# scenarios/VAE-2

Hardware: AMD Instinct MI355X
Metric: training frames/sec on 128x256 8-frame Cityscapes clips, 1/2/4/8 MI355X (higher is better)
Workload: dtype fp32; 1 GPU; VAE2 ELBO step (encz + encoder + 2 decoders fwd/bwd + Adam), HRNet-W18-small-v2, 128x256, 8 clips/GPU x 9 frames (CLIP_LENGTH=3); yaml=vae-2_amd/experiments/vae2_w18_small_v2_128x256.yaml, global_batch=8, frames_per_clip=9, parallelism=dp1, sync_bn=False, launch=hip_graph, mfma_operands=fp32

## Files before the change

### vae-2_amd/csrc/build.py

```python
import concurrent.futures as cf
import os
import shutil
import subprocess
import sys

HERE = os.path.dirname(os.path.abspath(__file__))
PKG = os.path.join(os.path.dirname(HERE), "vae2")
TAG = os.environ.get("VAE2_BUILD_TAG", "")
DEFS = os.environ.get("VAE2_DEFS", "").split()
OUT = os.path.join(PKG, f"libvae2_hip_{TAG}.so" if TAG else "libvae2_hip.so")
BUILD = os.path.join(HERE, f"build_{TAG}" if TAG else "build")
SOURCES = ["conv.hip", "bn.hip", "resample.hip", "elbo.hip", "heads.hip", "clips.hip",
           "metrics.hip", "wgrad_narrow.hip", "syncbn.hip", "dconv_stream.hip"]
HEADERS = ["common.h", os.path.join("..", "..", "include", "vae2_hip.h")]
ARCH = os.environ.get("VAE2_OFFLOAD_ARCH", "gfx950")
FLAGS = ["-O3", "-std=c++17", "-fPIC", f"--offload-arch={ARCH}", "-Wall",
         "-Wno-unused-function", "-munsafe-fp-atomics"]
EXTRA = {"conv.hip": ["-fno-slp-vectorize"], "dconv_stream.hip": ["-fno-slp-vectorize"]}
PARTS = {"conv.hip": 4}


def _units():
    out = []
    for src in SOURCES:
        n = PARTS.get(src, 0)
        base = os.path.splitext(src)[0]
        if n:
            out += [(src, f"{base}_p{i}.o", [f"-DVAE2_CONV_PART={i}"]) for i in range(n)]
        else:
            out.append((src, base + ".o", []))
    return out


def hipcc():
    for cand in (os.environ.get("HIPCC"), "/opt/rocm/bin/hipcc", shutil.which("hipcc")):
        if cand and os.path.exists(cand):
            return cand
    raise RuntimeError("hipcc not found (set HIPCC)")


def _newer(target, deps):
    if not os.path.exists(target):
        return True
    t = os.path.getmtime(target)
    return any(os.path.getmtime(d) > t for d in deps)


def _compile(unit):
    src, oname, defs = unit
    obj = os.path.join(BUILD, oname)
    deps = [os.path.join(HERE, src)] + [os.path.join(HERE, h) for h in HEADERS]
    if not _newer(obj, deps):
        return obj, None
    cmd = [hipcc()] + FLAGS + EXTRA.get(src, []) + defs + DEFS + ["-c", os.path.join(HERE, src), "-o", obj]
    r = subprocess.run(cmd, capture_output=True, text=True)
    if r.returncode != 0:
        return obj, f"$ {' '.join(cmd)}\n{r.stdout}\n{r.stderr}"
    return obj, None


def build(verbose=True, force=False):
    os.makedirs(BUILD, exist_ok=True)
    if force:
        for f in os.listdir(BUILD):
            os.remove(os.path.join(BUILD, f))
    units = _units()
    with cf.ThreadPoolExecutor(max_workers=min(8, len(units))) as ex:
        results = list(ex.map(_compile, units))
    errors = [e for _, e in results if e]
    if errors:
        raise RuntimeError("HIP compile failed:\n" + "\n".join(errors))
    objs = [o for o, _ in results]
    if force or _newer(OUT, objs):
        cmd = [hipcc(), "-shared", "-fPIC", f"--offload-arch={ARCH}", "-o", OUT] + objs
        r = subprocess.run(cmd, capture_output=True, text=True)
        if r.returncode != 0:
            raise RuntimeError(f"link failed:\n$ {' '.join(cmd)}\n{r.stdout}\n{r.stderr}")
    if verbose:
        print(f"built {OUT}")
    return OUT


if __name__ == "__main__":
    build(force="--force" in sys.argv)
```

### vae-2_amd/csrc/common.h

```cpp
#pragma once

#include <hip/hip_runtime.h>
#include <stdint.h>
#include <string>
#include <stdio.h>

#include "../../include/vae2_hip.h"

namespace vae2 {

constexpr int kSyncMaxRanks = 8;

void set_error(const std::string& msg);
int fail(const char* fn, const std::string& msg);
int check_launch(const char* fn);

void note_kernel(const void* host_fn);
#define VAE2_LAUNCH(K, ...)                                         \
  do {                                                              \
    ::vae2::note_kernel(reinterpret_cast<const void*>(K));          \
    hipLaunchKernelGGL(K, __VA_ARGS__);                             \
  } while (0)

#define VAE2_REQUIRE(cond, fn, msg)          \
// ... 95 lines not shown
inline int64_t act_pixels(const vae2_act* d) { return d->n * d->h * d->w; }
inline int64_t act_elems(const vae2_act* d) { return d->n * d->h * d->w * d->c; }

constexpr int kWave = 64;

__device__ __forceinline__ float wave_sum(float v) {
#pragma unroll
  for (int o = 32; o > 0; o >>= 1) v += __shfl_xor(v, o, 64);
  return v;
}

__device__ __forceinline__ double wave_sum_d(double v) {
#pragma unroll
  for (int o = 32; o > 0; o >>= 1) v += __shfl_xor(v, o, 64);
  return v;
}

inline int64_t ceil_div(int64_t a, int64_t b) { return (a + b - 1) / b; }

struct FastDiv {
  uint32_t d, m, s;
  FastDiv() : d(1), m(0), s(0) {}
  explicit FastDiv(uint32_t div) : d(div) {
    for (s = 0; s < 32; ++s)
      if ((1u << s) >= d) break;
    uint64_t one = 1;
    m = (uint32_t)(((one << 32) * ((one << s) - d)) / d + 1);
  }
  __device__ __forceinline__ uint32_t div(uint32_t n) const {
    return (__umulhi(n, m) + n) >> s;
  }
};

struct Lerp {
  int i0, i1;
  float l0, l1;
};

__device__ __forceinline__ Lerp lerp_index(int dst, int in_size, float scale) {
  float src = scale * ((float)dst + 0.5f) - 0.5f;
  if (src < 0.f) src = 0.f;
  int i0 = (int)src;
  if (i0 > in_size - 1) i0 = in_size - 1;
  int ip = (i0 < in_size - 1) ? 1 : 0;
  Lerp l;
  l.i0 = i0;
  l.i1 = i0 + ip;
  l.l1 = src - (float)i0;
  l.l0 = 1.f - l.l1;
  return l;
}

__device__ __forceinline__ float lerp_weight(int o, int in_size, float scale, int i) {
  Lerp l = lerp_index(o, in_size, scale);
  float w = 0.f;
  if (l.i0 == i) w += l.l0;
  if (l.i1 == i) w += l.l1;
  return w;
}

__device__ constexpr float hat_w(int d, int f) {
  return 1.f - (float)(2 * d + 1 - f < 0 ? f - 1 - 2 * d : 2 * d + 1 - f) / (float)(2 * f);
}

int adj3_fuse_launch(const float* dy, const vae2_act* dyd, int n, float* const* dxs,
                     const vae2_act* dxds, const float* betas, hipStream_t st);
extern int g_relu_dual_q;

int64_t wgrad3n_splits(const vae2_act* xd, const vae2_act* dyd);
int wgrad3n_launch(const float* x, const vae2_act* xd, const float* dy, const vae2_act* dyd,
                   float* part, const float* isave, int irelu, uint32_t x_bytes,
                   uint32_t dy_bytes, hipStream_t s);

extern int g_dconv_stream, g_dconv_stream_wpc, g_dconv_stream_bl, g_dconv_stream_spb,
    g_wgrad_narrow_tps, g_bn_blocks, g_bn_apply_res, g_fuse_quad;
bool dconv3s_shape(const vae2_act* ad, const vae2_act* yd);
int64_t dconv3s_rows(const vae2_act* ad, const vae2_act* yd);
int dconv3s_launch(const float* a, const vae2_act* ad, const float* wp, uint32_t w_bytes,
                   const float* bias, float* y, const vae2_act* yd, float beta, float* stats,
                   bool flip, const float* isave, int irelu, const float* bx, int bx_ps,
                   int brelu, const float* bsave, uint32_t bx_bytes, uint32_t a_bytes,
                   hipStream_t s);

int bias_grad_from_partials(const float* partials, int64_t rows, int64_t c,
                            float* dbias, int accumulate, void* stream);

inline unsigned ew_blocks(int64_t n, int threads = 256, int64_t cap = 65536) {
  int64_t b = ceil_div(n, threads);
  if (b > cap) b = cap;
  if (b < 1) b = 1;
  return (unsigned)b;
}

}
```

### vae-2_amd/csrc/conv.hip

```cpp
#include <mutex>
#include <vector>

#include "common.h"

#ifndef VAE2_ABLATE
#define VAE2_ABLATE 0
#endif

#ifndef VAE2_CONV_PART
#define VAE2_CONV_PART -1
#endif
#define VAE2_PART(n) (VAE2_CONV_PART < 0 || VAE2_CONV_PART == (n))

namespace vae2 {


static inline int round_up(int a, int b) { return (a + b - 1) / b * b; }

#if VAE2_PART(0)
__global__ void pack_weight_kernel(const float* __restrict__ w, int cout, int cin, int kk,
                                   int mode, int ld, float* __restrict__ out) {
  const int rows = mode == 0 ? (cout + 63) / 64 * 64 : (cin + 63) / 64 * 64;
  const int cols4 = mode == 0 ? (cin + 3) / 4 * 4 : (cout + 3) / 4 * 4;
  const int total = rows * kk * cols4;
// ... 2633 lines not shown
  const char* fn = "vae2_conv2d_pack_weight";
  VAE2_REQUIRE(w && out && cout > 0 && cin > 0 && k > 0 && (mode == 0 || mode == 1), fn,
               "bad arguments");
  VAE2_REQUIRE(ld >= cin * k * k && ld < (int64_t(1) << 31), fn, "bad row stride");
  int64_t total = vae2_conv2d_packed_size(cout, cin, k, mode);
  VAE2_LAUNCH(pack_weight_kernel, dim3(ew_blocks(total, 256, 2048)), dim3(256), 0,
                     as_stream(stream), w, (int)cout, (int)cin, k * k, mode, (int)ld, out);
  return check_launch(fn);
}

int vae2_conv2d_pack_weight(const float* w, int64_t cout, int64_t cin, int k, int mode,
                            float* out, void* stream) {
  return vae2_conv2d_pack_weight_ld(w, cout, cin, k, mode, cin * k * k, out, stream);
}

int vae2_conv2d_pack_weights(const vae2_pack_job* jobs, int64_t njobs, void* stream) {
  const char* fn = "vae2_conv2d_pack_weights";
  VAE2_REQUIRE(jobs && njobs > 0 && njobs <= 65535, fn, "bad job table");
  VAE2_LAUNCH(pack_weights_batched_kernel, dim3(32, (unsigned)njobs), dim3(256), 0,
                     as_stream(stream), jobs);
  return check_launch(fn);
}

int vae2_conv2d_set_tune(int key, int value) {
  if (key == 0) {
    const int prev = g_igemm_minblk;
    g_igemm_minblk = value < 0 ? 0 : value;
    return prev;
  }
  if (key == 1) {
    const int prev = g_wgrad_cols;
    g_wgrad_cols = value ? 1 : 0;
    return prev;
  }
  if (key == 2) {
    const int prev = g_dconv_nw8;
    g_dconv_nw8 = value ? 1 : 0;
    return prev;
  }
  if (key == 3) {
    const int prev = g_wgrad_nw8;
    g_wgrad_nw8 = value ? 1 : 0;
    return prev;
  }
  if (key == 4) {
    if (value < 3 || value > 8) return -1;
    const int prev = g_gemm1_tn;
    g_gemm1_tn = value;
    return prev;
  }
  if (key == 5) {
    const int prev = g_gemm1_tm;
    g_gemm1_tm = value == 1 ? 1 : 2;
    return prev;
  }
  if (key == 6) {
    if (value < 0 || value > 2) return -1;
    const int prev = g_igemm_nr;
    g_igemm_nr = value;
    return prev;
  }
  if (key == 8) {
    const int prev = g_bn_v2;
    g_bn_v2 = value ? 1 : 0;
    return prev;
  }
  if (key == 7) {
    if (value < 0 || value > 3) return -1;
    const int prev = g_wgrad_narrow;
    g_wgrad_narrow = value;
    return prev;
  }
  if (key == 9) {
    const int prev = g_dconv_stream;
    g_dconv_stream = value >= 0 && value <= 3 ? value : 3;
    return prev;
  }
  if (key == 18) {
    if (value < 256 || value > 8192) return -1;
    const int prev = g_wgrad_wgs;
    g_wgrad_wgs = value;
    return prev;
  }
  if (key == 21) {
    const int prev = g_fuse_quad;
    g_fuse_quad = value ? 1 : 0;
    return prev;
  }
  if (key == 20) {
    if (value < 0 || value > 65536) return -1;
    const int prev = g_bn_apply_res;
    g_bn_apply_res = value;
    return prev;
  }
  if (key == 19) {
    if (value < 256 || value > 8192) return -1;
    const int prev = g_bn_blocks;
    g_bn_blocks = value;
    return prev;
  }
  if (key == 16) {
    if (value < 1 || value > 2) return -1;
    const int prev = g_wgrad_narrow_tps;
    g_wgrad_narrow_tps = value;
    return prev;
  }
  if (key == 17) {
    if (value < 1 || value > 2) return -1;
    const int prev = g_dconv_stream_spb;
    g_dconv_stream_spb = value;
    return prev;
  }
  if (key == 15) {
    if (value < 0 || value > 2) return -1;
    const int prev = g_dconv_ksp;
    g_dconv_ksp = value;
    return prev;
  }
  if (key == 14) {
    const int prev = g_dconv_split72;
    g_dconv_split72 = value ? 1 : 0;
    return prev;
  }
  if (key == 13) {
    const int prev = g_dconv_n16;
    g_dconv_n16 = value ? 1 : 0;
    return prev;
  }
  if (key == 12) {
    const int prev = g_igemm_tab;
    g_igemm_tab = value ? 1 : 0;
    return prev;
  }
  if (key == 11) {
    const int prev = g_dconv_stream_bl;
    g_dconv_stream_bl = value ? 1 : 0;
    return prev;
  }
  if (key == 10) {
    const int prev = g_dconv_stream_wpc;
    g_dconv_stream_wpc = value >= 0 && value <= 8 ? value : 0;
    return prev;
  }
  return -1;
}

int vae2_conv2d_set_mfma_bf16(int on) {
  const int prev = g_bf16;
  g_bf16 = on ? 1 : 0;
  return prev;
}

#endif

#if VAE2_PART(3)
int vae2_wgrad_defer(int on) {
  const int prev = g_wr_defer ? 1 : 0;
  g_wr_defer = on != 0;
  return prev;
}

static int wgrad_flush_impl(void* stream, bool own_only) {
  const char* fn = "vae2_wgrad_flush";
  hipStream_t want = as_stream(stream);
  std::vector<WRQueued> q;
  {
    std::lock_guard<std::mutex> lk(g_wr_mu);
    if (own_only) {
      std::vector<WRQueued> keep;
      for (const WRQueued& j : g_wr_queue) (j.stream == want ? q : keep).push_back(j);
      g_wr_queue.swap(keep);
    } else {
      q.swap(g_wr_queue);
    }
  }
  size_t i = 0;
  while (i < q.size()) {
    WRMulti m{};
    hipStream_t st = want;
    int blocks = 0;
    while (i < q.size() && m.n < kWrMaxJobs) {
      WRJob j = q[i].job;
      const float* lo = j.dw;
      const float* hi = j.dw + (int64_t)(j.cout - 1) * j.ld + (int64_t)j.cin * j.k * j.k;
      bool clash = false;
      for (int u = 0; u < m.n; ++u) {
        const float* lo2 = m.j[u].dw;
        const float* hi2 = m.j[u].dw + (int64_t)(m.j[u].cout - 1) * m.j[u].ld +
                           (int64_t)m.j[u].cin * m.j[u].k * m.j[u].k;
        if (lo < hi2 && lo2 < hi) clash = true;
      }
      if (clash) break;
      j.blk0 = blocks;
      blocks += (int)ceil_div((int64_t)j.cout * j.k * j.k * j.cin4, 32);
      m.j[m.n++] = j;
      ++i;
    }
    VAE2_LAUNCH(wgrad_reduce_multi_kernel, dim3((unsigned)blocks), dim3(256), 0, st, m);
    const int rc = check_launch(fn);
    if (rc) return rc;
  }
  return 0;
}

int vae2_wgrad_flush(void* stream) { return wgrad_flush_impl(stream, false); }

int vae2_wgrad_flush_stream(void* stream) { return wgrad_flush_impl(stream, true); }



#endif

#if VAE2_PART(0)
int vae2_conv2d_set_algo(int algo) {
  const int prev = g_conv_algo + (g_wide_tiles ? 0 : 4) + (g_ksplit ? 0 : 8) +
                   (g_dconv_nr ? 0 : 16) + (g_gemm1 ? 0 : 32) + (g_vec_out ? 0 : 64) +
                   (g_dconv_nr_wide ? 0 : 128);
  const int a = algo & 7;
  if (algo >= 0 && algo <= 255 && a <= 6 && a != 3) {
    g_dconv_nr_wide = (algo & 128) ? 0 : 1;
    g_conv_algo = a & 3;
    g_wide_tiles = a < 4;
    g_ksplit = !(algo & 8);
    g_dconv_nr = !(algo & 16);
    g_gemm1 = !(algo & 32);
    g_vec_out = !(algo & 64);
  }
  return prev;
}

int64_t vae2_conv2d_fwd_stats_rows(const float* x, const vae2_act* xd, const vae2_act* yd,
                                   int k, int stride, int pad) {
  if (!act_ok(xd) || !act_ok(yd)) return 0;
  if (dconv_use(xd, yd, k, stride, pad, x)) return dconv_rows(xd, yd);
  G1Tile g1;
  if (gemm1_pick(xd, yd, k, stride, pad, x, &g1)) return g1.grid_x;
  return igemm_rows(act_pixels(yd), (int)yd->c, k * k, round_up((int)xd->c, 4));
}

int vae2_conv2d_fwd_kernel_name(const vae2_act* xd, const vae2_act* yd, int k, int stride,
                                int pad, char* buf, int64_t len) {
  if (!xd || !yd || !buf || len <= 0) return -22;
  if (dconv_use(xd, yd, k, stride, pad, (const float*)16)) {
    if (stream_use(xd, yd)) {
      const int q = (int)((xd->c + 3) / 4);
      snprintf(buf, (size_t)len, "dconv3s_kernel<%d, %d, %d, false", q == 5 ? 1 : 2,
               q == 5 ? 2 : 4, q);
      return 0;
    }
    DTile d = pick_dtile(xd, yd);
    if (d.nr)
      snprintf(buf, (size_t)len, "dconv3_kernel<%d, %d, false, false, %d>", d.tm, d.tn, d.nr);
    else
      snprintf(buf, (size_t)len, "dconv3_kernel<%d, %d, false>", d.tm, d.tn);
    return 0;
  }
  G1Tile g1;
  if (gemm1_pick(xd, yd, k, stride, pad, (const float*)16, &g1)) {
    snprintf(buf, (size_t)len, "gemm1x1_kernel<%d, %d>", g1.tm, g1.tn);
    return 0;
  }
  Tile t = pick_igemm_tile(act_pixels(yd), (int)yd->c, k * k, round_up((int)xd->c, 4), 1);
  if (t.ks > 1)
    snprintf(buf, (size_t)len, "igemm_kernel<%d, %d, true, 0, %d>", t.tm, t.tn, t.ks);
  else
    snprintf(buf, (size_t)len, "igemm_kernel<%d, %d, true, 0>", t.tm, t.tn);
  return 0;
}

int vae2_conv2d_fwd(const float* x, const vae2_act* xd, const float* wp,
                    const float* bias, float* y, const vae2_act* yd, int k,
                    int stride, int pad, float beta, float* stats,
                    void* stream) {
  const char* fn = "vae2_conv2d_fwd";
  VAE2_REQUIRE(x && wp && y, fn, "null pointer");
  VAE2_REQUIRE(conv_shapes_ok(xd, yd, k, stride, pad), fn, "inconsistent conv shapes");
  VAE2_REQUIRE(fits32(xd) && fits32(yd), fn, "tensor too large for 32-bit indexing");
  if (dconv_use(xd, yd, k, stride, pad, x)) {
    return launch_dconv(x, xd, wp, (uint32_t)(vae2_conv2d_packed_size(yd->c, xd->c, k, 0) * 4),
                        bias, y, yd, beta, stats, false, as_stream(stream), fn);
  }
  G1Tile g1;
  if (gemm1_pick(xd, yd, k, stride, pad, x, &g1)) {
    const int rc = launch_gemm1(x, xd, wp,
                                (uint32_t)(vae2_conv2d_packed_size(yd->c, xd->c, k, 0) * 4),
                                bias, y, yd, beta, stats, g1, as_stream(stream), fn);
    if (rc != -1) return rc;
    VAE2_REQUIRE(stats == nullptr, fn, "BN statistics need a 16-byte aligned output here");
  }
  IGemm p{};
  p.a = x; p.a_ps = (int)xd->ps; p.a_c = (int)xd->c; p.a_c4 = round_up((int)xd->c, 4);
  p.a_h = (int)xd->h; p.a_w = (int)xd->w;
  p.g_n = (int)yd->n; p.g_h = (int)yd->h; p.g_w = (int)yd->w;
  p.a_step = stride;
  p.nth = k; p.ntw = k;
  p.dh0 = -pad; p.dhs = 1; p.dw0 = -pad; p.dws = 1;
  p.kh0 = 0; p.khs = 1; p.kw0 = 0; p.kws = 1; p.ksz = k;
  p.w = wp; p.n = (int)yd->c;
  p.a_bytes = act_bytes(xd);
  p.w_bytes = (uint32_t)(vae2_conv2d_packed_size(yd->c, xd->c, k, 0) * 4);
  p.bias = bias;
  p.y = y; p.y_ps = (int)yd->ps; p.y_h = (int)yd->h; p.y_w = (int)yd->w;
  p.y_step = 1; p.y_offh = 0; p.y_offw = 0;
  p.beta = beta;
  p.stats = stats;
  return launch_igemm(p, 0, as_stream(stream), fn);
}

int vae2_conv2d_bnin_ok(const float* x, const vae2_act* xd, const vae2_act* yd, int k,
                        int stride, int pad) {
  if (!x || !conv_shapes_ok(xd, yd, k, stride, pad) || !fits32(xd) || !fits32(yd)) return 0;
  return !g_bf16 && dconv_use(xd, yd, k, stride, pad, x) && g_conv_algo != 1 &&
         wgrad3_shape_ok(xd, yd, k, stride, pad) && vec_ok(x, (int)xd->ps);
}

int vae2_conv2d_fwd_bnin(const float* x, const vae2_act* xd, const float* bn_save, int relu,
                         const float* wp, const float* bias, float* y, const vae2_act* yd,
                         int k, int stride, int pad, float beta, float* stats, void* stream) {
  const char* fn = "vae2_conv2d_fwd_bnin";
  VAE2_REQUIRE(x && wp && y && bn_save, fn, "null pointer");
  VAE2_REQUIRE(conv_shapes_ok(xd, yd, k, stride, pad), fn, "inconsistent conv shapes");
  VAE2_REQUIRE(vae2_conv2d_bnin_ok(x, xd, yd, k, stride, pad), fn,
               "input BatchNorm needs the direct 3x3 kernels (vae2_conv2d_bnin_ok)");
  BnSide bn;
  bn.isave = bn_save;
  bn.irelu = relu ? 1 : 0;
  return launch_dconv(x, xd, wp, (uint32_t)(vae2_conv2d_packed_size(yd->c, xd->c, k, 0) * 4),
                      bias, y, yd, beta, stats, false, as_stream(stream), fn, bn);
}

static int igemm_dgrad_setup(IGemm& p, const float* dy, const vae2_act* dyd, const float* wp,
                             float* dx, const vae2_act* dxd, int k, int stride, int pad,
                             float beta);
static int64_t igemm_dgrad_rows(const float* dy, const vae2_act* dyd, const vae2_act* dxd,
                                int k, int stride, int pad);

int64_t vae2_conv2d_bwd_data_bnpart_rows(const float* dy, const vae2_act* dyd,
                                         const vae2_act* dxd, int k, int stride, int pad) {
  if (!dy || !conv_shapes_ok(dxd, dyd, k, stride, pad) || !fits32(dxd) || !fits32(dyd))
    return 0;
  if (g_bf16) return 0;
  if (dconv_use(dyd, dxd, k, stride, pad, dy)) return dconv_rows(dyd, dxd);
  G1Tile g1;
  if (gemm1_pick(dyd, dxd, k, stride, pad, dy, &g1)) return g1.grid_x;
  return igemm_dgrad_rows(dy, dyd, dxd, k, stride, pad);
}

int vae2_conv2d_bwd_data_bnpart(const float* dy, const vae2_act* dyd, const float* wp,
                                float* dx, const vae2_act* dxd, int k, int stride, int pad,
                                const float* bn_x, const vae2_act* bn_xd, const float* bn_save,
                                int relu, float* partials, void* stream) {
  const char* fn = "vae2_conv2d_bwd_data_bnpart";
  VAE2_REQUIRE(dy && wp && dx && bn_x && bn_xd && bn_save && partials, fn, "null pointer");
  VAE2_REQUIRE(conv_shapes_ok(dxd, dyd, k, stride, pad), fn, "inconsistent conv shapes");
  VAE2_REQUIRE(bn_xd->n == dxd->n && bn_xd->h == dxd->h && bn_xd->w == dxd->w &&
               bn_xd->c == dxd->c && bn_xd->ps >= bn_xd->c && fits32(bn_xd), fn,
               "BatchNorm input shape must match dx");
  VAE2_REQUIRE(vae2_conv2d_bwd_data_bnpart_rows(dy, dyd, dxd, k, stride, pad) > 0, fn,
               "BatchNorm partials are not available for this geometry "
               "(vae2_conv2d_bwd_data_bnpart_rows)");
  const uint32_t wbytes = (uint32_t)(vae2_conv2d_packed_size(dyd->c, dxd->c, k, 1) * 4);
  if (dconv_use(dyd, dxd, k, stride, pad, dy)) {
    BnSide bn;
    bn.bx = bn_x;
    bn.bx_ps = (int)bn_xd->ps;
    bn.bx_bytes = act_bytes(bn_xd);
    bn.bsave = bn_save;
    bn.brelu = relu ? 1 : 0;
    return launch_dconv(dy, dyd, wp, wbytes, nullptr, dx, dxd, 0.f, partials, true,
                        as_stream(stream), fn, bn);
  }
  G1Tile g1;
  if (gemm1_pick(dyd, dxd, k, stride, pad, dy, &g1)) {
    const int rc = launch_gemm1(dy, dyd, wp, wbytes, nullptr, dx, dxd, 0.f, partials, g1,
                                as_stream(stream), fn, bn_x, (int)bn_xd->ps, relu ? 1 : 0,
                                bn_save, act_bytes(bn_xd));
    VAE2_REQUIRE(rc != -1, fn, "1x1 GEMM refused the partials form");
    return rc;
  }
  IGemm p{};
  const int ncls = igemm_dgrad_setup(p, dy, dyd, wp, dx, dxd, k, stride, pad, 0.f);
  VAE2_REQUIRE(ncls > 0, fn, "stride > 2 is not supported");
  p.stats = partials;
  p.bx = bn_x;
  p.bx_ps = (int)bn_xd->ps;
  p.bx_bytes = act_bytes(bn_xd);
  p.bsave = bn_save;
  p.brelu = relu ? 1 : 0;
  return launch_igemm(p, 1, as_stream(stream), fn, ncls);
}

int vae2_conv2d_bwd_data(const float* dy, const vae2_act* dyd, const float* wp,
                         float* dx, const vae2_act* dxd, int k, int stride,
                         int pad, float beta, void* stream) {
  const char* fn = "vae2_conv2d_bwd_data";
  VAE2_REQUIRE(dy && wp && dx, fn, "null pointer");
  VAE2_REQUIRE(conv_shapes_ok(dxd, dyd, k, stride, pad), fn, "inconsistent conv shapes");
  VAE2_REQUIRE(fits32(dxd) && fits32(dyd), fn, "tensor too large for 32-bit indexing");
  if (dconv_use(dyd, dxd, k, stride, pad, dy))
    return launch_dconv(dy, dyd, wp, (uint32_t)(vae2_conv2d_packed_size(dyd->c, dxd->c, k, 1) * 4),
                        nullptr, dx, dxd, beta, nullptr, true, as_stream(stream), fn);
  G1Tile g1;
  if (gemm1_pick(dyd, dxd, k, stride, pad, dy, &g1)) {
    const int rc = launch_gemm1(dy, dyd, wp,
                                (uint32_t)(vae2_conv2d_packed_size(dyd->c, dxd->c, k, 1) * 4),
                                nullptr, dx, dxd, beta, nullptr, g1, as_stream(stream), fn);
    if (rc != -1) return rc;
  }
  IGemm p{};
  const int ncls = igemm_dgrad_setup(p, dy, dyd, wp, dx, dxd, k, stride, pad, beta);
  VAE2_REQUIRE(ncls >= 0, fn, "stride > 2 is not supported");
  if (ncls == 0) return 0;
  return launch_igemm(p, 1, as_stream(stream), fn, ncls);
}

static int igemm_dgrad_setup(IGemm& p, const float* dy, const vae2_act* dyd, const float* wp,
                             float* dx, const vae2_act* dxd, int k, int stride, int pad,
                             float beta) {
  p.a = dy; p.a_ps = (int)dyd->ps; p.a_c = (int)dyd->c; p.a_c4 = round_up((int)dyd->c, 4);
  p.a_h = (int)dyd->h; p.a_w = (int)dyd->w;
  p.g_n = (int)dxd->n;
  p.a_step = 1;
  p.dhs = -1; p.dws = -1;
  p.khs = stride; p.kws = stride; p.ksz = k;
  p.w = wp; p.n = (int)dxd->c;
  p.a_bytes = act_bytes(dyd);
  p.w_bytes = (uint32_t)(vae2_conv2d_packed_size(dyd->c, dxd->c, k, 1) * 4);
  p.bias = nullptr;
  p.y = dx; p.y_ps = (int)dxd->ps; p.y_h = (int)dxd->h; p.y_w = (int)dxd->w;
  p.y_step = stride;
  p.beta = beta;
  p.stats = nullptr;
  int ncls = 0;
  for (int ph = 0; ph < stride; ++ph) {
    for (int pw = 0; pw < stride; ++pw) {
      int gh = (int)((dxd->h - ph + stride - 1) / stride);
      int gw = (int)((dxd->w - pw + stride - 1) / stride);
      if (gh <= 0 || gw <= 0) continue;
      if (ncls >= 4) return -1;
      int kh0 = ((ph + pad) % stride + stride) % stride;
      int kw0 = ((pw + pad) % stride + stride) % stride;
      int nth = kh0 < k ? (k - 1 - kh0) / stride + 1 : 0;
      int ntw = kw0 < k ? (k - 1 - kw0) / stride + 1 : 0;
      IGemm::Cls& c = p.cls[ncls++];
      c.g_h = gh; c.g_w = gw;
      c.nth = nth; c.ntw = ntw;
      c.dh0 = (ph + pad - kh0) / stride;
      c.dw0 = (pw + pad - kw0) / stride;
      c.kh0 = kh0; c.kw0 = kw0;
      c.y_offh = ph; c.y_offw = pw;
      if (nth == 0 || ntw == 0) { c.nth = 0; c.ntw = 1; }
    }
  }
  if (ncls == 0) return 0;
  {
    const IGemm::Cls& c = p.cls[0];
    p.g_h = c.g_h; p.g_w = c.g_w; p.nth = c.nth; p.ntw = c.ntw;
    p.dh0 = c.dh0; p.dw0 = c.dw0; p.kh0 = c.kh0; p.kw0 = c.kw0;
    p.y_offh = c.y_offh; p.y_offw = c.y_offw;
  }
  return ncls;
}

static int64_t igemm_dgrad_rows(const float* dy, const vae2_act* dyd, const vae2_act* dxd,
                                int k, int stride, int pad) {
  IGemm p{};
  const int ncls = igemm_dgrad_setup(p, dy, dyd, nullptr, nullptr, dxd, k, stride, pad, 0.f);
  if (ncls <= 0) return 0;
  int64_t M = (int64_t)p.g_n * p.g_h * p.g_w;
  int max_taps = p.nth * p.ntw;
  for (int c = 0; c < ncls && ncls > 1; ++c) {
    const IGemm::Cls& q = p.cls[c];
    const int64_t mc = (int64_t)p.g_n * q.g_h * q.g_w;
    if (mc > M) M = mc;
    if (q.nth * q.ntw > max_taps) max_taps = q.nth * q.ntw;
  }
  const Tile t = pick_igemm_tile(M, p.n, max_taps, p.a_c4, ncls);
  return ceil_div(M, igemm_rows_per_block(t)) * ncls;
}

#endif
// ... 248 lines not shown
```

### vae-2_amd/vae2/prof.py

```python
import ctypes
import re
from collections import defaultdict

import torch

from . import _lib

_ACTIVE = None

FAMILIES = (
    ("conv_fwd", r"dconv3_(group_)?kernel<\d+, \d+, false|dconv3s_kernel<\d+, \d+, \d+, false|"
                 r"igemm_kernel<\d+, \d+, \w+, 0"),
    ("conv_dgrad", r"dconv3_(group_)?kernel<\d+, \d+, true|dconv3s_kernel<\d+, \d+, \d+, true|"
                   r"igemm_kernel<\d+, \d+, \w+, [12]"),
    ("conv_wgrad", r"wgrad"),
    ("conv_1x1", r"gemm1x1"),
    ("batchnorm", r"bn_|reduce_then|chan_partials|partials_reduce"),
    ("heads", r"upsum|head_|up_adj"),
    ("fuse_resample", r"upsample|fuse_sum|relu_bwd|copy_act|tile_kernel|spatial_|codemap"),
    ("optimizer", r"adam|sgd|grad_sumsq|clip_coeffs|clip_scale|pack_weight"),
    ("loss_elbo", r"l1_|reparam|weighted_sum|finish_sum|scale_kernel|nonfinite|nchw|nhwc|"
                  r"sqdiff"),
    ("torch_aten", r"at::native|^at::"),
    ("copies", r"rocclr_copy|rocclr_fill"),
)

FP32_MFMA_PEAK_TF = 157.3
BF16_MFMA_PEAK_TF = 2500.0
HBM_PEAK_GBS = 8000.0
MFMA_PEAK_TF = FP32_MFMA_PEAK_TF


def set_mfma_dtype(dtype):
    global MFMA_PEAK_TF
    MFMA_PEAK_TF = BF16_MFMA_PEAK_TF if dtype == "bf16" else FP32_MFMA_PEAK_TF


def family(kernel):
    for f, rx in FAMILIES:
        if re.search(rx, kernel):
            return f
    return "other"


_ABI_FAMILY = (("conv_dgrad", "bwd_data"), ("conv_wgrad", "bwd_weight"), ("conv_fwd", "conv2d"),
               ("heads", "head_|upsum"), ("batchnorm", "bn_"))


def _abi_family(name):
    for f, key in _ABI_FAMILY:
        if re.search(key, name):
            return f
    return "other"


def active():
    return _ACTIVE


def note(flops=0.0, nbytes=0.0, shape=None):
    if _ACTIVE is not None:
        if _ACTIVE.pending is not None:
            _ACTIVE.conflicts += 1
        _ACTIVE.pending = (float(flops), float(nbytes), shape)


def take():
    if _ACTIVE is None:
        return None
    w, _ACTIVE.pending = _ACTIVE.pending, None
    return w


def put(work):
    if _ACTIVE is not None and work is not None:
        if _ACTIVE.pending is not None:
            _ACTIVE.conflicts += 1
        _ACTIVE.pending = work


def conv_label(kind, cin, cout, k, stride, h, w):
    return f"{kind} {cin}->{cout} k{k} s{stride} @{h}x{w}"


def fwd_kernel_name(xa, yshape, k, stride, pad):
    buf = ctypes.create_string_buffer(64)
    n, oh, ow, cout = yshape
    y = _lib.Act(n, oh, ow, cout, cout)
    _lib.check(_lib.load().vae2_conv2d_fwd_kernel_name(ctypes.byref(xa), ctypes.byref(y), k,
                                                       stride, pad, buf, 64))
    return buf.value.decode()


_SLEEP_RATE = {}


def _sleep_cycles(us):
# ... 127 lines not shown
```

Before: 922.1 frames/s.

## Add dedicated direct stride-2 3x3 conv kernel for forward and dgrad

Adds a new direct convolution kernel specialised for 3x3 stride-2 pad-1 convs with small channel counts, used for both forward and data-gradient paths. The input patch is staged in LDS with an even/odd column split for the forward pass, and dgrad is decomposed into four output-parity classes with precomputed tap tables. It fuses bias, BatchNorm statistic partials and ReLU-masked BN backward partials into the epilogue. The kernel only runs for a whitelist of channel geometries and replaces the generic dconv/igemm paths there, at the cost of another large kernel and extra dispatch complexity.

```diff
diff --git a/vae-2_amd/csrc/build.py b/vae-2_amd/csrc/build.py
--- a/vae-2_amd/csrc/build.py
+++ b/vae-2_amd/csrc/build.py
@@ -11,12 +11,13 @@
 OUT = os.path.join(PKG, f"libvae2_hip_{TAG}.so" if TAG else "libvae2_hip.so")
 BUILD = os.path.join(HERE, f"build_{TAG}" if TAG else "build")
 SOURCES = ["conv.hip", "bn.hip", "resample.hip", "elbo.hip", "heads.hip", "clips.hip",
-           "metrics.hip", "wgrad_narrow.hip", "syncbn.hip", "dconv_stream.hip"]
+           "metrics.hip", "wgrad_narrow.hip", "syncbn.hip", "dconv_stream.hip", "dconv_s2.hip"]
 HEADERS = ["common.h", os.path.join("..", "..", "include", "vae2_hip.h")]
 ARCH = os.environ.get("VAE2_OFFLOAD_ARCH", "gfx950")
 FLAGS = ["-O3", "-std=c++17", "-fPIC", f"--offload-arch={ARCH}", "-Wall",
          "-Wno-unused-function", "-munsafe-fp-atomics"]
-EXTRA = {"conv.hip": ["-fno-slp-vectorize"], "dconv_stream.hip": ["-fno-slp-vectorize"]}
+EXTRA = {"conv.hip": ["-fno-slp-vectorize"], "dconv_stream.hip": ["-fno-slp-vectorize"],
+         "dconv_s2.hip": ["-fno-slp-vectorize"]}
 PARTS = {"conv.hip": 4}
 
 
diff --git a/vae-2_amd/csrc/common.h b/vae-2_amd/csrc/common.h
--- a/vae-2_amd/csrc/common.h
+++ b/vae-2_amd/csrc/common.h
@@ -201,6 +201,16 @@
                    int brelu, const float* bsave, uint32_t bx_bytes, uint32_t a_bytes,
                    hipStream_t s);
 
+extern int g_dconv_s2;
+int64_t dconv_s2_rows(const float* a, const vae2_act* xd, const vae2_act* yd, int k, int stride,
+                      int pad, bool dgrad);
+int dconv_s2_name(const vae2_act* xd, const vae2_act* yd, int k, int stride, int pad, char* buf,
+                  int64_t len);
+int dconv_s2_launch(const float* a, const vae2_act* xd, const vae2_act* yd, const float* wp,
+                    uint32_t w_bytes, uint32_t a_bytes, const float* bias, float* out, float beta,
+                    float* stats, bool dgrad, const float* bx, int bx_ps, int brelu,
+                    const float* bsave, uint32_t bx_bytes, hipStream_t st, const char* fn);
+
 int bias_grad_from_partials(const float* partials, int64_t rows, int64_t c,
                             float* dbias, int accumulate, void* stream);
 
diff --git a/vae-2_amd/csrc/conv.hip b/vae-2_amd/csrc/conv.hip
--- a/vae-2_amd/csrc/conv.hip
+++ b/vae-2_amd/csrc/conv.hip
@@ -2739,6 +2739,12 @@
     g_wgrad_wgs = value;
     return prev;
   }
+  if (key == 22) {
+    if (value < 0 || value > 3) return -1;
+    const int prev = g_dconv_s2;
+    g_dconv_s2 = value;
+    return prev;
+  }
   if (key == 21) {
     const int prev = g_fuse_quad;
     g_fuse_quad = value ? 1 : 0;
@@ -2889,6 +2895,7 @@
 int64_t vae2_conv2d_fwd_stats_rows(const float* x, const vae2_act* xd, const vae2_act* yd,
                                    int k, int stride, int pad) {
   if (!act_ok(xd) || !act_ok(yd)) return 0;
+  if (const int64_t r2 = dconv_s2_rows(x, xd, yd, k, stride, pad, false)) return r2;
   if (dconv_use(xd, yd, k, stride, pad, x)) return dconv_rows(xd, yd);
   G1Tile g1;
   if (gemm1_pick(xd, yd, k, stride, pad, x, &g1)) return g1.grid_x;
@@ -2898,6 +2905,8 @@
 int vae2_conv2d_fwd_kernel_name(const vae2_act* xd, const vae2_act* yd, int k, int stride,
                                 int pad, char* buf, int64_t len) {
   if (!xd || !yd || !buf || len <= 0) return -22;
+  if (dconv_s2_rows((const float*)16, xd, yd, k, stride, pad, false))
+    return dconv_s2_name(xd, yd, k, stride, pad, buf, len);
   if (dconv_use(xd, yd, k, stride, pad, (const float*)16)) {
     if (stream_use(xd, yd)) {
       const int q = (int)((xd->c + 3) / 4);
@@ -2933,6 +2942,11 @@
   VAE2_REQUIRE(x && wp && y, fn, "null pointer");
   VAE2_REQUIRE(conv_shapes_ok(xd, yd, k, stride, pad), fn, "inconsistent conv shapes");
   VAE2_REQUIRE(fits32(xd) && fits32(yd), fn, "tensor too large for 32-bit indexing");
+  if (dconv_s2_rows(x, xd, yd, k, stride, pad, false))
+    return dconv_s2_launch(x, xd, yd, wp,
+                           (uint32_t)(vae2_conv2d_packed_size(yd->c, xd->c, k, 0) * 4),
+                           act_bytes(xd), bias, y, beta, stats, false, nullptr, 0, 0, nullptr, 0,
+                           as_stream(stream), fn);
   if (dconv_use(xd, yd, k, stride, pad, x)) {
     return launch_dconv(x, xd, wp, (uint32_t)(vae2_conv2d_packed_size(yd->c, xd->c, k, 0) * 4),
                         bias, y, yd, beta, stats, false, as_stream(stream), fn);
@@ -2997,6 +3011,7 @@
   if (!dy || !conv_shapes_ok(dxd, dyd, k, stride, pad) || !fits32(dxd) || !fits32(dyd))
     return 0;
   if (g_bf16) return 0;
+  if (const int64_t r2 = dconv_s2_rows(dy, dxd, dyd, k, stride, pad, true)) return r2;
   if (dconv_use(dyd, dxd, k, stride, pad, dy)) return dconv_rows(dyd, dxd);
   G1Tile g1;
   if (gemm1_pick(dyd, dxd, k, stride, pad, dy, &g1)) return g1.grid_x;
@@ -3017,6 +3032,10 @@
                "BatchNorm partials are not available for this geometry "
                "(vae2_conv2d_bwd_data_bnpart_rows)");
   const uint32_t wbytes = (uint32_t)(vae2_conv2d_packed_size(dyd->c, dxd->c, k, 1) * 4);
+  if (dconv_s2_rows(dy, dxd, dyd, k, stride, pad, true))
+    return dconv_s2_launch(dy, dxd, dyd, wp, wbytes, act_bytes(dyd), nullptr, dx, 0.f, partials,
+                           true, bn_x, (int)bn_xd->ps, relu ? 1 : 0, bn_save, act_bytes(bn_xd),
+                           as_stream(stream), fn);
   if (dconv_use(dyd, dxd, k, stride, pad, dy)) {
     BnSide bn;
     bn.bx = bn_x;
@@ -3054,6 +3073,11 @@
   VAE2_REQUIRE(dy && wp && dx, fn, "null pointer");
   VAE2_REQUIRE(conv_shapes_ok(dxd, dyd, k, stride, pad), fn, "inconsistent conv shapes");
   VAE2_REQUIRE(fits32(dxd) && fits32(dyd), fn, "tensor too large for 32-bit indexing");
+  if (dconv_s2_rows(dy, dxd, dyd, k, stride, pad, true))
+    return dconv_s2_launch(dy, dxd, dyd, wp,
+                           (uint32_t)(vae2_conv2d_packed_size(dyd->c, dxd->c, k, 1) * 4),
+                           act_bytes(dyd), nullptr, dx, beta, nullptr, true, nullptr, 0, 0,
+                           nullptr, 0, as_stream(stream), fn);
   if (dconv_use(dyd, dxd, k, stride, pad, dy))
     return launch_dconv(dy, dyd, wp, (uint32_t)(vae2_conv2d_packed_size(dyd->c, dxd->c, k, 1) * 4),
                         nullptr, dx, dxd, beta, nullptr, true, as_stream(stream), fn);
diff --git a/vae-2_amd/csrc/dconv_s2.hip b/vae-2_amd/csrc/dconv_s2.hip
--- /dev/null
+++ b/vae-2_amd/csrc/dconv_s2.hip
@@ -0,0 +1,498 @@
+#include "common.h"
+
+namespace vae2 {
+
+extern int g_bf16, g_conv_algo, g_vec_out;
+int g_dconv_s2 = 3;
+
+constexpr int kS2Tab = 384;
+constexpr int kS2ClsTab = 96;
+constexpr int kS2MaxC4 = 76;
+
+struct DS2 {
+  const float* a;
+  int a_ps, a_c, a_c4, a_h, a_w;
+  int tiles_h, tiles_w;
+  int csp;
+  int csplit;
+  const float* w;
+  uint32_t a_bytes, w_bytes;
+  int n;
+  const float* bias;
+  float* y;
+  int y_ps, y_h, y_w;
+  float beta;
+  float* stats;
+  int vec_out;
+  const float* bx;
+  int bx_ps, brelu;
+  const float* bsave;
+  uint32_t bx_bytes;
+};
+
+template <int TN, int NR, int ROLE>
+__global__ __launch_bounds__(256) void dconv_s2_kernel(DS2 p) {
+  extern __shared__ __attribute__((aligned(16))) float tile[];
+  constexpr int BN = 16 * TN, BNT = BN + NR;
+  __shared__ float red[4][2][BNT];
+  const int NT = blockDim.x, NW = NT >> 6;
+  const int lane = threadIdx.x & 63, wave = threadIdx.x >> 6;
+  const int g = lane >> 4, r = lane & 15;
+  const int bm = xcd_remap(blockIdx.x, gridDim.x);
+  const int per_img = p.tiles_h * p.tiles_w;
+  const int img = bm / per_img;
+  const int trem = bm - img * per_img;
+  const int th = trem / p.tiles_w, tw = trem - th * p.tiles_w;
+  const int n0 = blockIdx.y * BNT;
+  const int kk4 = 9 * p.a_c4, Q = p.a_c4 >> 2, csp = p.csp;
+  const int NRP = ROLE == 0 ? NW >> 1 : (p.csplit ? NW >> 2 : NW);
+  const int LH = ROLE == 0 ? NW + 1 : NRP + 1, LW = ROLE == 0 ? 65 : 17;
+  const int oh0 = th * (ROLE == 0 ? NRP : 2 * NRP), ow0 = tw * 32;
+  const int sh0 = ROLE == 0 ? 2 * oh0 - 1 : oh0 >> 1, sw0 = ROLE == 0 ? 2 * ow0 - 1 : ow0 >> 1;
+  const int zoff = LH * LW * csp;
+  int2* const tab = reinterpret_cast<int2*>(tile + zoff + 4);
+
+  const __amdgpu_buffer_rsrc_t arsrc = make_rsrc(p.a, p.a_bytes);
+  const __amdgpu_buffer_rsrc_t wrsrc = make_rsrc(p.w, p.w_bytes);
+
+  constexpr int SB = 7;
+  const int sq = threadIdx.x % Q, pb = threadIdx.x / Q, pstride = NT / Q;
+  const int sc = sq * 4;
+  const bool cpad = sc + 4 > p.a_c;
+  const int npix = LH * LW;
+  auto issue = [&](int pix0, f4* v) {
+#pragma unroll
+    for (int u = 0; u < SB; ++u) {
+      const int pix = pix0 + u * pstride;
+      const int lr = pix / LW, lc = pix - lr * LW;
+      const int ih = sh0 + lr, iw = sw0 + lc;
+      const bool ok = pix < npix && (unsigned)ih < (unsigned)p.a_h && (unsigned)iw < (unsigned)p.a_w;
+      v[u] = load4(arsrc, ok ? (uint32_t)((((int64_t)img * p.a_h + ih) * p.a_w + iw) * p.a_ps + sc) * 4u
+                             : kOOB);
+    }
+  };
+  auto commit = [&](int pix0, f4* v) {
+#pragma unroll
+    for (int u = 0; u < SB; ++u) {
+      const int pix = pix0 + u * pstride;
+      if (pix >= npix) break;
+      if (cpad) {
+#pragma unroll
+        for (int k = 0; k < 4; ++k)
+          if (sc + k >= p.a_c) v[u][k] = 0.f;
+      }
+      int slot = pix;
+      if (ROLE == 0) {
+        const int lr = pix / LW, lc = pix - lr * LW;
+        slot = lr * LW + ((lc & 1) ? 33 + (lc >> 1) : lc >> 1);
+      }
+      *reinterpret_cast<f4*>(&tile[slot * csp + 4 * sq]) = v[u];
+    }
+  };
+  f4 sv[SB];
+  int spix = pb < pstride ? pb : npix;
+  issue(spix, sv);
+
+  for (int e = threadIdx.x; e < kS2Tab; e += NT) {
+    int aoff = 0;
+    uint32_t woff = kOOB;
+    if (ROLE == 0) {
+      const int t = e / Q, q = e - t * Q;
+      if (t < 9) {
+        const int kh = t / 3, kw = t - 3 * kh;
+        aoff = (kh * LW + (kw == 1 ? 33 : kw >> 1)) * csp + 4 * q;
+        woff = (uint32_t)(t * p.a_c4 + 4 * q) * 4u;
+      }
+    } else {
+      const int cls = e / kS2ClsTab, k = e - cls * kS2ClsTab;
+      const int ph = cls >> 1, pw = cls & 1;
+      const int ntw = pw ? 2 : 1, ntaps = (ph ? 2 : 1) * ntw;
+      const int t = k / Q, q = k - t * Q;
+      if (t < ntaps) {
+        const int i = t / ntw, j = t - i * ntw;
+        const int kh = (ph ? 0 : 1) + 2 * i, kw = (pw ? 0 : 1) + 2 * j;
+        aoff = ((ph - i) * LW + (pw - j)) * csp + 4 * q;
+        woff = (uint32_t)((kh * 3 + kw) * p.a_c4 + 4 * q) * 4u;
+      }
+    }
+    tab[e] = make_int2(aoff, (int)woff);
+  }
+  if (threadIdx.x < 4) tile[zoff + threadIdx.x] = 0.f;
+
+  commit(spix, sv);
+  for (spix += SB * pstride; spix < npix; spix += SB * pstride) {
+    issue(spix, sv);
+    commit(spix, sv);
+  }
+  __syncthreads();
+
+  uint32_t wrow[TN];
+#pragma unroll
+  for (int j = 0; j < TN; ++j) wrow[j] = (uint32_t)((n0 + j * 16 + r) * kk4) * 4u;
+  uint32_t wrowr[NR > 0 ? NR : 1];
+#pragma unroll
+  for (int q = 0; q < NR; ++q) wrowr[q] = (uint32_t)((n0 + BN + q) * kk4) * 4u;
+
+  const bool bnp = ROLE == 1 && p.bx != nullptr;
+  float csum[TN], csq[TN], bmn[TN], bis[TN], bsc[TN], bsh[TN];
+#pragma unroll
+  for (int j = 0; j < TN; ++j) {
+    csum[j] = 0.f; csq[j] = 0.f;
+    const int n = n0 + j * 16 + r < p.n ? n0 + j * 16 + r : p.n - 1;
+    bmn[j] = bnp ? p.bsave[n] : 0.f;
+    bis[j] = bnp ? p.bsave[p.n + n] : 0.f;
+    bsc[j] = bnp ? p.bsave[2 * p.n + n] : 0.f;
+    bsh[j] = bnp ? p.bsave[3 * p.n + n] : 0.f;
+  }
+  float rsum[NR > 0 ? NR : 1], rsq[NR > 0 ? NR : 1];
+#pragma unroll
+  for (int q = 0; q < NR; ++q) { rsum[q] = 0.f; rsq[q] = 0.f; }
+
+  auto run = [&](const int2* tab0, const int nch, const int abase, const int oh, const int owb,
+                 const int ows) {
+    constexpr int D = 2;
+    f4 acc[TN], fa[D], fb[D][TN], fr[D][NR > 0 ? NR : 1];
+    float racc[NR > 0 ? NR : 1];
+#pragma unroll
+    for (int j = 0; j < TN; ++j) acc[j] = f4{0.f, 0.f, 0.f, 0.f};
+#pragma unroll
+    for (int q = 0; q < NR; ++q) racc[q] = 0.f;
+    int kc = g;
+    auto load = [&](f4& fa, f4* fb, f4* fr) {
+      const int2 e = tab0[kc];
+      kc += 4;
+      const uint32_t woff = (uint32_t)e.y;
+      fa = *reinterpret_cast<const f4*>(&tile[woff == kOOB ? zoff : abase + e.x]);
+#pragma unroll
+      for (int j = 0; j < TN; ++j) fb[j] = load4(wrsrc, wrow[j] + woff);
+#pragma unroll
+      for (int q = 0; q < NR; ++q) fr[q] = load4(wrsrc, woff == kOOB ? kOOB : wrowr[q] + woff);
+    };
+    auto mma = [&](const f4& fa, const f4* fb, const f4* fr) {
+#pragma unroll
+      for (int s = 0; s < 4; ++s)
+#pragma unroll
+        for (int j = 0; j < TN; ++j)
+          acc[j] = __builtin_amdgcn_mfma_f32_16x16x4f32(fa[s], fb[j][s], acc[j], 0, 0, 0);
+#pragma unroll
+      for (int q = 0; q < NR; ++q)
+#pragma unroll
+        for (int s = 0; s < 4; ++s) racc[q] = __builtin_fmaf(fa[s], fr[q][s], racc[q]);
+    };
+#pragma unroll
+    for (int d = 0; d < D - 1; ++d) load(fa[d], fb[d], fr[d]);
+    for (int ch = 0; ch < nch; ch += D) {
+#pragma unroll
+      for (int d = 0; d < D; ++d) {
+        load(fa[(d + D - 1) % D], fb[(d + D - 1) % D], fr[(d + D - 1) % D]);
+        mma(fa[d], fb[d], fr[d]);
+      }
+    }
+
+    const bool rowok = oh < p.y_h;
+    const int64_t rowpix = ((int64_t)img * p.y_h + (rowok ? oh : 0)) * p.y_w;
+    if (p.vec_out) {
+      const int k = r & 3, qc = 4 * (r >> 2);
+      if (p.stats && bnp) {
+        const __amdgpu_buffer_rsrc_t bxr = make_rsrc(p.bx, p.bx_bytes);
+        float xv[4][TN];
+#pragma unroll
+        for (int e = 0; e < 4; ++e) {
+          const int ow = owb + (g * 4 + e) * ows;
+          const bool pin = rowok && ow < p.y_w;
+#pragma unroll
+          for (int j = 0; j < TN; ++j) {
+            const int n = n0 + j * 16 + r;
+            xv[e][j] = load1(bxr, pin && n < p.n ? (uint32_t)(((rowpix + ow) * p.bx_ps + n) * 4) : kOOB);
+          }
+        }
+#pragma unroll
+        for (int e = 0; e < 4; ++e) {
+          const int ow = owb + (g * 4 + e) * ows;
+          const bool pin = rowok && ow < p.y_w;
+#pragma unroll
+          for (int j = 0; j < TN; ++j) {
+            const int n = n0 + j * 16 + r;
+            const float v = acc[j][e];
+            const float x = xv[e][j];
+            const float gv = (p.brelu && !(__builtin_fmaf(x, bsc[j], bsh[j]) > 0.f)) ? 0.f : v;
+            const bool ok = pin && n < p.n;
+            csum[j] += ok ? gv : 0.f;
+            csq[j] += ok ? gv * (x - bmn[j]) * bis[j] : 0.f;
+          }
+        }
+      } else if (p.stats) {
+#pragma unroll
+        for (int e = 0; e < 4; ++e) {
+          const int ow = owb + (g * 4 + e) * ows;
+          if (!rowok || ow >= p.y_w) continue;
+#pragma unroll
+          for (int j = 0; j < TN; ++j) {
+            const int n = n0 + j * 16 + r;
+            if (n >= p.n) continue;
+            const float v = acc[j][e] + (p.bias ? p.bias[n] : 0.f);
+            csum[j] += v;
+            csq[j] += v * v;
+          }
+        }
+      }
+      const int ow = owb + (g * 4 + k) * ows;
+      const bool pok = rowok && ow < p.y_w;
+      float* yrow = p.y + (rowpix + (pok ? ow : 0)) * p.y_ps;
+      f4 yold[TN];
+      if (p.beta != 0.f) {
+#pragma unroll
+        for (int j = 0; j < TN; ++j) {
+          const int n = n0 + j * 16 + qc;
+          yold[j] = (pok && n + 3 < p.n) ? *reinterpret_cast<const f4*>(yrow + n)
+                                         : f4{0.f, 0.f, 0.f, 0.f};
+        }
+      }
+#pragma unroll
+      for (int j = 0; j < TN; ++j) {
+        f4 v = acc[j];
+        quad_transpose(v, k);
+        const int n = n0 + j * 16 + qc;
+        if (!pok || n >= p.n) continue;
+        if (p.bias) {
+#pragma unroll
+          for (int q = 0; q < 4; ++q) v[q] += n + q < p.n ? p.bias[n + q] : 0.f;
+        }
+        if (n + 3 < p.n) {
+          if (p.beta != 0.f) v += p.beta * yold[j];
+          *reinterpret_cast<f4*>(yrow + n) = v;
+        } else {
+#pragma unroll
+          for (int q = 0; q < 4; ++q)
+            if (n + q < p.n) yrow[n + q] = p.beta != 0.f ? v[q] + p.beta * yrow[n + q] : v[q];
+        }
+      }
+    } else {
+#pragma unroll
+      for (int e = 0; e < 4; ++e) {
+        const int ow = owb + (g * 4 + e) * ows;
+        if (!rowok || ow >= p.y_w) continue;
+        float* yrow = p.y + (rowpix + ow) * p.y_ps;
+        const float* xrow = bnp ? p.bx + (rowpix + ow) * p.bx_ps : nullptr;
+#pragma unroll
+        for (int j = 0; j < TN; ++j) {
+          const int n = n0 + j * 16 + r;
+          if (n >= p.n) continue;
+          float v = acc[j][e];
+          if (p.bias) v += p.bias[n];
+          if (p.beta != 0.f) v += p.beta * yrow[n];
+          yrow[n] = v;
+          if (bnp) {
+            const float x = xrow[n];
+            const float gv = (p.brelu && !(__builtin_fmaf(x, bsc[j], bsh[j]) > 0.f)) ? 0.f : v;
+            csum[j] += gv;
+            csq[j] += gv * (x - bmn[j]) * bis[j];
+          } else {
+            csum[j] += v;
+            csq[j] += v * v;
+          }
+        }
+      }
+    }
+    if constexpr (NR > 0) {
+#pragma unroll
+      for (int q = 0; q < NR; ++q) {
+        racc[q] += __shfl_xor(racc[q], 16, 64);
+        racc[q] += __shfl_xor(racc[q], 32, 64);
+      }
+#pragma unroll
+      for (int q = 0; q < NR; ++q) {
+        if ((q & 3) != g) continue;
+        const int n = n0 + BN + q;
+        const int ow = owb + r * ows;
+        const bool mok = rowok && ow < p.y_w && n < p.n;
+        const int nc = n < p.n ? n : p.n - 1;
+        float* yp = p.y + (rowpix + (mok ? ow : 0)) * p.y_ps + nc;
+        float v = racc[q];
+        if (p.bias) v += p.bias[nc];
+        if (p.beta != 0.f && mok) v += p.beta * *yp;
+        if (mok) *yp = v;
+        if (bnp) {
+          const __amdgpu_buffer_rsrc_t bxr = make_rsrc(p.bx, p.bx_bytes);
+          const float x = load1(bxr, mok ? (uint32_t)(((rowpix + ow) * p.bx_ps + n) * 4) : kOOB);
+          const float gv =
+              (p.brelu && !(__builtin_fmaf(x, p.bsave[2 * p.n + nc], p.bsave[3 * p.n + nc]) > 0.f))
+                  ? 0.f : v;
+          rsum[q] += mok ? gv : 0.f;
+          rsq[q] += mok ? gv * (x - p.bsave[nc]) * p.bsave[p.n + nc] : 0.f;
+        } else {
+          rsum[q] += mok ? v : 0.f;
+          rsq[q] += mok ? v * v : 0.f;
+        }
+      }
+    }
+  };
+
+  if constexpr (ROLE == 0) {
+    const int orow = wave >> 1, ocol = (wave & 1) * 16;
+    run(tab, (9 * Q + 3) >> 2, (orow * 2 * LW + ocol + r) * csp, oh0 + orow, ow0 + ocol, 1);
+  } else {
+    const int rp = p.csplit ? wave >> 2 : wave;
+    const int c0 = p.csplit ? wave & 3 : 0, c1 = p.csplit ? c0 + 1 : 4;
+#pragma unroll 1
+    for (int cls = c0; cls < c1; ++cls) {
+      const int ph = cls >> 1, pw = cls & 1;
+      const int ntaps = (ph ? 2 : 1) * (pw ? 2 : 1);
+      run(tab + cls * kS2ClsTab, (ntaps * Q + 3) >> 2, (rp * LW + r) * csp,
+          oh0 + 2 * rp + ph, ow0 + pw, 2);
+    }
+  }
+
+  if (p.stats) {
+#pragma unroll
+    for (int j = 0; j < TN; ++j) {
+      csum[j] += __shfl_xor(csum[j], 16, 64);
+      csum[j] += __shfl_xor(csum[j], 32, 64);
+      csq[j] += __shfl_xor(csq[j], 16, 64);
+      csq[j] += __shfl_xor(csq[j], 32, 64);
+    }
+    if (g == 0) {
+#pragma unroll
+      for (int j = 0; j < TN; ++j) {
+        red[wave][0][j * 16 + r] = csum[j];
+        red[wave][1][j * 16 + r] = csq[j];
+      }
+    }
+    if constexpr (NR > 0) {
+#pragma unroll
+      for (int q = 0; q < NR; ++q) {
+#pragma unroll
+        for (int o = 1; o < 16; o <<= 1) {
+          rsum[q] += __shfl_xor(rsum[q], o, 64);
+          rsq[q] += __shfl_xor(rsq[q], o, 64);
+        }
+      }
+      if (r == 0) {
+#pragma unroll
+        for (int q = 0; q < NR; ++q) {
+          if ((q & 3) != g) continue;
+          red[wave][0][BN + q] = rsum[q];
+          red[wave][1][BN + q] = rsq[q];
+        }
+      }
+    }
+    __syncthreads();
+    const int rows = gridDim.x;
+    for (int c = threadIdx.x; c < BNT; c += NT) {
+      if (n0 + c >= p.n) continue;
+      float s = red[0][0][c], s2 = red[0][1][c];
+      for (int w = 1; w < NW; ++w) {
+        s += red[w][0][c];
+        s2 += red[w][1][c];
+      }
+      p.stats[(int64_t)bm * p.n + n0 + c] = s;
+      p.stats[((int64_t)rows + bm) * p.n + n0 + c] = s2;
+    }
+  }
+}
+
+namespace {
+
+struct S2Plan {
+  int nw, tn, nr, nblk, tiles_h, tiles_w, csp, csplit;
+  int64_t tiles;
+  size_t lds;
+};
+
+size_t s2_lds(int rows, int csp, bool dgrad) {
+  return ((size_t)rows * (dgrad ? 17 : 65) * csp + 4) * sizeof(float) + kS2Tab * sizeof(int2);
+}
+
+bool s2_plan(const float* a, const vae2_act* ad, const vae2_act* od, int k, int stride, int pad,
+             bool dgrad, S2Plan* out) {
+  if (k != 3 || stride != 2 || pad != 1 || g_bf16) return false;
+  if ((uintptr_t)a % 16 != 0 || ad->ps % 4 != 0) return false;
+  const int c4 = ((int)ad->c + 3) / 4 * 4, N = (int)od->c;
+  if (c4 > kS2MaxC4 || N > 1024) return false;
+  S2Plan s;
+  s.csp = ((c4 >> 2) & 1) ? c4 : c4 + 4;
+  if (N == 18) {
+    s.tn = 1; s.nr = 2; s.nblk = 1;
+  } else {
+    const int t16 = (N + 15) / 16;
+    s.nblk = (t16 + 3) / 4;
+    s.tn = (t16 + s.nblk - 1) / s.nblk;
+    s.nr = 0;
+  }
+  s.csplit = 0;
+  for (int pass = 0; pass < 2; ++pass) {
+    s.nw = dgrad || pass == 0 ? 4 : 2;
+    s.csplit = dgrad && pass == 1;
+    const int bh = dgrad ? (s.csplit ? 2 : 8) : s.nw / 2;
+    s.tiles_h = (int)ceil_div(od->h, bh);
+    s.tiles_w = (int)ceil_div(od->w, 32);
+    s.tiles = od->n * s.tiles_h * s.tiles_w;
+    s.lds = s2_lds(dgrad ? bh / 2 + 1 : s.nw + 1, s.csp, dgrad);
+    if (s.lds <= 64 * 1024 && (pass == 1 || s.tiles * s.nblk >= 512)) break;
+    if (pass == 1) return false;
+  }
+  if (s.tiles > 0x7fffffff) return false;
+  if (out) *out = s;
+  return true;
+}
+
+bool s2_listed(const vae2_act* xd, const vae2_act* yd, bool dgrad) {
+  if (act_pixels(yd) < 16384) return false;
+  if (!dgrad) return xd->c == 36 && yd->c == 72;
+  return (xd->c == 18 || xd->c == 36) && (yd->c == 18 || yd->c == 36 || yd->c == 72);
+}
+
+template <int ROLE>
+void s2_launch_tn(const DS2& p, const S2Plan& s, dim3 grid, hipStream_t st) {
+  const dim3 blk(64 * s.nw);
+  if (s.nr == 2) VAE2_LAUNCH((dconv_s2_kernel<1, 2, ROLE>), grid, blk, s.lds, st, p);
+  else if (s.tn == 1) VAE2_LAUNCH((dconv_s2_kernel<1, 0, ROLE>), grid, blk, s.lds, st, p);
+  else if (s.tn == 2) VAE2_LAUNCH((dconv_s2_kernel<2, 0, ROLE>), grid, blk, s.lds, st, p);
+  else if (s.tn == 3) VAE2_LAUNCH((dconv_s2_kernel<3, 0, ROLE>), grid, blk, s.lds, st, p);
+  else VAE2_LAUNCH((dconv_s2_kernel<4, 0, ROLE>), grid, blk, s.lds, st, p);
+}
+
+}
+
+int64_t dconv_s2_rows(const float* a, const vae2_act* xd, const vae2_act* yd, int k, int stride,
+                      int pad, bool dgrad) {
+  if (g_conv_algo == 1 || !((g_dconv_s2 >> (dgrad ? 1 : 0)) & 1)) return 0;
+  S2Plan s;
+  if (!s2_plan(a, dgrad ? yd : xd, dgrad ? xd : yd, k, stride, pad, dgrad, &s)) return 0;
+  if (g_conv_algo != 2 && !s2_listed(xd, yd, dgrad)) return 0;
+  return s.tiles;
+}
+
+int dconv_s2_name(const vae2_act* xd, const vae2_act* yd, int k, int stride, int pad, char* buf,
+                  int64_t len) {
+  S2Plan s;
+  if (!s2_plan((const float*)16, xd, yd, k, stride, pad, false, &s)) return -1;
+  snprintf(buf, (size_t)len, "dconv_s2_kernel<%d, %d, 0>", s.tn, s.nr);
+  return 0;
+}
+
+int dconv_s2_launch(const float* a, const vae2_act* xd, const vae2_act* yd, const float* wp,
+                    uint32_t w_bytes, uint32_t a_bytes, const float* bias, float* out, float beta,
+                    float* stats, bool dgrad, const float* bx, int bx_ps, int brelu,
+                    const float* bsave, uint32_t bx_bytes, hipStream_t st, const char* fn) {
+  const vae2_act* ad = dgrad ? yd : xd;
+  const vae2_act* od = dgrad ? xd : yd;
+  S2Plan s;
+  if (!s2_plan(a, ad, od, 3, 2, 1, dgrad, &s)) return fail(fn, "not a stride-2 direct geometry");
+  DS2 p{};
+  p.a = a; p.a_ps = (int)ad->ps; p.a_c = (int)ad->c; p.a_c4 = ((int)ad->c + 3) / 4 * 4;
+  p.a_h = (int)ad->h; p.a_w = (int)ad->w;
+  p.tiles_h = s.tiles_h; p.tiles_w = s.tiles_w; p.csp = s.csp; p.csplit = s.csplit;
+  p.w = wp; p.a_bytes = a_bytes; p.w_bytes = w_bytes;
+  p.n = (int)od->c; p.bias = bias;
+  p.y = out; p.y_ps = (int)od->ps; p.y_h = (int)od->h; p.y_w = (int)od->w;
+  p.beta = beta; p.stats = stats;
+  p.vec_out = g_vec_out && (uintptr_t)out % 16 == 0 && od->ps % 4 == 0 && !(stats && beta != 0.f);
+  p.bx = bx; p.bx_ps = bx_ps; p.brelu = brelu; p.bsave = bsave; p.bx_bytes = bx_bytes;
+  const dim3 grid((unsigned)s.tiles, (unsigned)s.nblk);
+  if (dgrad) s2_launch_tn<1>(p, s, grid, st);
+  else s2_launch_tn<0>(p, s, grid, st);
+  return check_launch(fn);
+}
+
+}
diff --git a/vae-2_amd/vae2/prof.py b/vae-2_amd/vae2/prof.py
--- a/vae-2_amd/vae2/prof.py
+++ b/vae-2_amd/vae2/prof.py
@@ -10,9 +10,9 @@
 
 FAMILIES = (
     ("conv_fwd", r"dconv3_(group_)?kernel<\d+, \d+, false|dconv3s_kernel<\d+, \d+, \d+, false|"
-                 r"igemm_kernel<\d+, \d+, \w+, 0"),
+                 r"igemm_kernel<\d+, \d+, \w+, 0|dconv_s2_kernel<\d+, \d+, 0"),
     ("conv_dgrad", r"dconv3_(group_)?kernel<\d+, \d+, true|dconv3s_kernel<\d+, \d+, \d+, true|"
-                   r"igemm_kernel<\d+, \d+, \w+, [12]"),
+                   r"igemm_kernel<\d+, \d+, \w+, [12]|dconv_s2_kernel<\d+, \d+, 1"),
     ("conv_wgrad", r"wgrad"),
     ("conv_1x1", r"gemm1x1"),
     ("batchnorm", r"bn_|reduce_then|chan_partials|partials_reduce"),
```

Result: no change. 925.6 frames/s, median of 6 (+0.4%).
